# ShinYwings/SingleHDR-tf2

Hardware: AMD Instinct MI355X
Metric: HDR images/sec (512x512) end-to-end inference, deq+lin+hal (higher is better)
Workload: dtype f32

## Files before the change

### include/shdr.h

```cpp
#ifndef SHDR_H_
#define SHDR_H_

#include <stdint.h>

#ifdef __cplusplus
extern "C" {
#endif

void shdr_config_reload(void);

#define SHDR_OK          0
#define SHDR_E_SHAPE    (-1)
#define SHDR_E_ALIGN    (-2)
#define SHDR_E_ARCH     (-3)
#define SHDR_E_LAUNCH   (-4)
#define SHDR_E_NULL     (-5)

#define SHDR_ACT_NONE   0
#define SHDR_ACT_RELU   1
#define SHDR_ACT_LRELU  2
#define SHDR_ACT_TANH   3

#define SHDR_ALGO_AUTO    0
#define SHDR_ALGO_MFMA    1
// ... 55 lines not shown
int shdr_conv2d_plan_f32(const shdr_conv2d_desc* d, int has_residual);
int64_t shdr_conv2d_prepared_filter_elems_f32(const shdr_conv2d_desc* d, int has_residual);
int shdr_conv2d_filter_is_plain_f32(const shdr_conv2d_desc* d, int has_residual);
int shdr_conv2d_prepare_filter_f32(const shdr_conv2d_desc* d, int has_residual, const float* w, float* prepared, void* stream);
int64_t shdr_conv2d_workspace_bytes_f32(const shdr_conv2d_desc* d, int has_residual);
int shdr_conv2d_fwd_prepared_f32(const shdr_conv2d_desc* d, const float* x1, const float* x2, const float* prepared,
                                 const float* bias, const float* scale, const float* shift, const float* residual, float* y,
                                 float* y_pool, void* workspace, void* stream);
int shdr_conv2d_fwd_prepared_ranged_f32(const shdr_conv2d_desc* d, const float* x1, const float* x2, const float* prepared,
                                        const float* bias, const float* scale, const float* shift, const float* residual, float* y,
                                        float* y_pool, void* workspace, const float* x1_range, const float* x2_range, float* y_range,
                                        void* stream);
int shdr_conv2d_projected_ok_f32(const shdr_conv2d_desc* d);
int shdr_conv2d_fwd_prepared_projected_f32(const shdr_conv2d_desc* d, const float* x1, const float* x2, const float* prepared,
                                           const float* bias, const float* scale, const float* shift, const float* proj, float* y_proj,
                                           float* y, float* y_pool, void* workspace, const float* x1_range, const float* x2_range,
                                           float* y_range, void* stream);

int shdr_conv2d_up2_lowres_ok_f32(const shdr_conv2d_desc* d);
int64_t shdr_conv2d_up2_lowres_filter_elems_f32(const shdr_conv2d_desc* d);
int shdr_conv2d_up2_lowres_prepare_filter_f32(const shdr_conv2d_desc* d, const float* w, float* prepared, void* stream);
int64_t shdr_conv2d_up2_lowres_workspace_bytes_f32(const shdr_conv2d_desc* d);
int shdr_conv2d_fwd_up2_lowres_f32(const shdr_conv2d_desc* d, const float* x, const float* prepared, const float* bias,
                                   const float* scale, const float* shift, float* y, void* workspace, const float* x_range,
                                   float* y_range, void* stream);

int shdr_conv2d_up2_fused_ok_f32(const shdr_conv2d_desc* d);
int shdr_conv2d_up2_narrow_enabled(void);
int64_t shdr_conv2d_up2_fused_filter_elems_f32(const shdr_conv2d_desc* d);
int shdr_conv2d_up2_fused_prepare_filter_f32(const shdr_conv2d_desc* d, const float* w, float* prepared, void* stream);
int shdr_conv2d_fwd_up2_fused_f32(const shdr_conv2d_desc* d, const float* x, const float* prepared, const float* bias,
                                  const float* scale, const float* shift, const float* proj, float* y_proj, float* y,
                                  const float* x_range, float* y_range, void* stream);

int shdr_conv2d_wgrad_f32(const shdr_conv2d_desc* d, const float* x, int which, const float* dz,
                          float* dw, void* stream);
int shdr_filter_transform_f32(const float* w, float* wt, int KH, int KW, int Cin, int Cout,
                              int c_begin, int c_count, float scale, void* stream);
int64_t shdr_conv2d_dgrad_workspace_bytes_f32(const shdr_conv2d_desc* d, int which);
int shdr_conv2d_dgrad_f32(const shdr_conv2d_desc* d, int which, const float* dz, const float* w, float* dx, void* workspace,
                          void* stream);
int shdr_conv2d_dgrad_tracks_range_f32(const shdr_conv2d_desc* d, int which);
int shdr_conv2d_dgrad_ranged_f32(const shdr_conv2d_desc* d, int which, const float* dz, const float* w, float* dx, void* workspace,
                                 const float* dz_range, float* dx_range, void* stream);
enum { SHDR_OP_CONV2D_FWD = 0, SHDR_OP_CONV2D_DGRAD = 1, SHDR_OP_CONV2D_WGRAD_WINOGRAD = 2, SHDR_OP_BATCHNORM = 3,
       SHDR_OP_ACT_BWD_BIAS = 4  };
#define SHDR_BN_MAX_BLOCKS 1024
int64_t shdr_workspace_bytes(int op, const shdr_conv2d_desc* d, int arg);
int shdr_bias_grad_f32(const float* dz, float* db, int64_t npix, int C, void* stream);

int shdr_soft_hist_fwd_f32(const float* x, float* y, int64_t npix, int C, int B, void* stream);
int shdr_soft_hist_bwd_f32(const float* x, const float* dy, float* dx, int64_t npix, int C, int B, void* stream);

int shdr_lin_frontend_fwd_f32(const float* img, float* y, int N, int H, int W,
                              int y_channels, void* stream);

int shdr_avgpool2_fwd_f32(const float* x, float* y, int N, int H, int W, int C, void* stream);
int shdr_maxpool2_fwd_f32(const float* x, float* y, int N, int H, int W, int C, void* stream);
int shdr_maxpool3s2_fwd_f32(const float* x, float* y, int N, int H, int W, int C, void* stream);
int shdr_resize2x_fwd_f32(const float* x, float* y, int N, int H, int W, int C, void* stream);
int shdr_gap_fwd_f32(const float* x, float* y, int N, int HW, int C, void* stream);

int shdr_invcrf_decode_fwd_f32(const float* feat, const float* wfc, const float* bfc,
                               const float* table, float* out, int B, int F, int K,
                               void* stream);
int shdr_increase_fwd_f32(const float* rf, float* out, int B, int K, void* stream);
// ... 457 lines not shown
```

### singlehdr-tf2_amd/_lib.py

```python
import ctypes
import os

_HERE = os.path.dirname(os.path.abspath(__file__))
LIB_PATH = os.environ.get("SHDR_LIB") or os.path.join(_HERE, "libshdr.so")

c_int = ctypes.c_int
c_i64 = ctypes.c_int64
c_f32 = ctypes.c_float
c_ptr = ctypes.c_void_p


class ConvDesc(ctypes.Structure):
    _fields_ = [("N", ctypes.c_int32), ("H", ctypes.c_int32), ("W", ctypes.c_int32),
                ("C1", ctypes.c_int32), ("C2", ctypes.c_int32),
                ("Cout", ctypes.c_int32), ("KH", ctypes.c_int32), ("KW", ctypes.c_int32),
                ("stride", ctypes.c_int32), ("pad_t", ctypes.c_int32), ("pad_l", ctypes.c_int32),
                ("Ho", ctypes.c_int32), ("Wo", ctypes.c_int32),
                ("x2_scale", ctypes.c_float),
                ("act1", ctypes.c_int32), ("act2", ctypes.c_int32),
                ("res_cstride", ctypes.c_int32), ("y_cstride", ctypes.c_int32),
                ("algo", ctypes.c_int32), ("cout_valid", ctypes.c_int32),
                ("w_batch_stride", ctypes.c_int64),
                ("y_pix_stride", ctypes.c_int32), ("y_off_h", ctypes.c_int32), ("y_off_w", ctypes.c_int32),
                ("y_H", ctypes.c_int32), ("y_W", ctypes.c_int32),
# ... 72 lines not shown
    "shdr_config_reload": (None, []),
    "shdr_conv2d_x3_input_absmax_f32": (c_int, [c_ptr, c_i64, c_ptr, c_ptr]),
    "shdr_conv2d_x3n_ok_f32": (c_int, [ctypes.POINTER(ConvDesc)]),
    "shdr_conv2d_x3n_filter_elems_f32": (c_i64, [ctypes.POINTER(ConvDesc)]),
    "shdr_conv2d_x3n_prepare_filter_f32": (c_int, [ctypes.POINTER(ConvDesc), c_ptr, c_ptr, c_ptr]),
    "shdr_conv2d_fwd_x3n_f32": (c_int, [ctypes.POINTER(ConvDesc)] + [c_ptr] * 10),
    "shdr_conv2d_fwd_x3n_ranged_f32": (c_int, [ctypes.POINTER(ConvDesc)] + [c_ptr] * 13),
    "shdr_act_bwd_bias_f32": (c_int, [c_ptr, c_ptr, c_ptr, c_ptr, c_ptr, c_i64, c_int, c_int, c_ptr]),
    "shdr_winograd_filter_packed_f32": (c_int, [c_ptr, c_ptr, c_int, c_int, c_ptr]),
    "shdr_conv2d_wgrad_winograd_f32": (c_int, [c_ptr] * 4 + [c_int] * 7 + [c_f32, c_ptr]),
    "shdr_crc32c": (ctypes.c_uint32, [c_ptr, ctypes.c_uint64, ctypes.c_uint32]),
    "shdr_same_pad": (c_int, [c_int, c_int, c_int, ctypes.POINTER(c_int), ctypes.POINTER(c_int)]),
    "shdr_conv2d_fwd_f32": (c_int, [ctypes.POINTER(ConvDesc)] + [c_ptr] * 9),
    "shdr_conv2d_fwd_yrange_f32": (c_int, [ctypes.POINTER(ConvDesc)] + [c_ptr] * 10),
    "shdr_conv2d_plan_f32": (c_int, [ctypes.POINTER(ConvDesc), c_int]),
    "shdr_conv2d_prepared_filter_elems_f32": (c_i64, [ctypes.POINTER(ConvDesc), c_int]),
    "shdr_conv2d_filter_is_plain_f32": (c_int, [ctypes.POINTER(ConvDesc), c_int]),
    "shdr_conv2d_prepare_filter_f32": (c_int, [ctypes.POINTER(ConvDesc), c_int, c_ptr, c_ptr, c_ptr]),
    "shdr_conv2d_workspace_bytes_f32": (c_i64, [ctypes.POINTER(ConvDesc), c_int]),
    "shdr_conv2d_fwd_prepared_f32": (c_int, [ctypes.POINTER(ConvDesc)] + [c_ptr] * 11),
    "shdr_conv2d_fwd_prepared_ranged_f32": (c_int, [ctypes.POINTER(ConvDesc)] + [c_ptr] * 14),
    "shdr_conv2d_projected_ok_f32": (c_int, [ctypes.POINTER(ConvDesc)]),
    "shdr_conv2d_fwd_prepared_projected_f32": (c_int, [ctypes.POINTER(ConvDesc)] + [c_ptr] * 15),
    "shdr_conv2d_up2_lowres_ok_f32": (c_int, [ctypes.POINTER(ConvDesc)]),
    "shdr_conv2d_up2_lowres_filter_elems_f32": (c_i64, [ctypes.POINTER(ConvDesc)]),
    "shdr_conv2d_up2_lowres_prepare_filter_f32": (c_int, [ctypes.POINTER(ConvDesc), c_ptr, c_ptr, c_ptr]),
    "shdr_conv2d_up2_lowres_workspace_bytes_f32": (c_i64, [ctypes.POINTER(ConvDesc)]),
    "shdr_conv2d_fwd_up2_lowres_f32": (c_int, [ctypes.POINTER(ConvDesc)] + [c_ptr] * 10),
    "shdr_conv2d_up2_fused_ok_f32": (c_int, [ctypes.POINTER(ConvDesc)]),
    "shdr_conv2d_up2_narrow_enabled": (c_int, []),
    "shdr_conv2d_up2_fused_filter_elems_f32": (c_i64, [ctypes.POINTER(ConvDesc)]),
    "shdr_conv2d_up2_fused_prepare_filter_f32": (c_int, [ctypes.POINTER(ConvDesc), c_ptr, c_ptr, c_ptr]),
    "shdr_conv2d_fwd_up2_fused_f32": (c_int, [ctypes.POINTER(ConvDesc)] + [c_ptr] * 11),
    "shdr_conv2d_fwd_x3_projected_f32": (c_int, [ctypes.POINTER(ConvDesc)] + [c_ptr] * 14),
    "shdr_conv2d_fwd_x3_residual_f32": (c_int, [ctypes.POINTER(ConvDesc)] + [c_ptr] * 12),
    "shdr_conv2d_dgrad_workspace_bytes_f32": (c_i64, [ctypes.POINTER(ConvDesc), c_int]),
    "shdr_conv2d_dgrad_f32": (c_int, [ctypes.POINTER(ConvDesc), c_int, c_ptr, c_ptr, c_ptr, c_ptr, c_ptr]),
    "shdr_conv2d_dgrad_tracks_range_f32": (c_int, [ctypes.POINTER(ConvDesc), c_int]),
    "shdr_conv2d_dgrad_ranged_f32": (c_int, [ctypes.POINTER(ConvDesc), c_int, c_ptr, c_ptr, c_ptr, c_ptr, c_ptr, c_ptr, c_ptr]),
    "shdr_workspace_bytes": (c_i64, [c_int, ctypes.POINTER(ConvDesc), c_int]),
    "shdr_soft_hist_bwd_f32": (c_int, [c_ptr, c_ptr, c_ptr, c_i64, c_int, c_int, c_ptr]),
    "shdr_conv2d_wgrad_f32": (c_int, [ctypes.POINTER(ConvDesc), c_ptr, c_int, c_ptr, c_ptr, c_ptr]),
    "shdr_filter_transform_f32": (c_int, [c_ptr, c_ptr, c_int, c_int, c_int, c_int, c_int, c_int, c_f32, c_ptr]),
    "shdr_bias_grad_f32": (c_int, [c_ptr, c_ptr, c_i64, c_int, c_ptr]),
    "shdr_soft_hist_fwd_f32": (c_int, [c_ptr, c_ptr, c_i64, c_int, c_int, c_ptr]),
    "shdr_lin_frontend_fwd_f32": (c_int, [c_ptr, c_ptr, c_int, c_int, c_int, c_int, c_ptr]),
    "shdr_avgpool2_fwd_f32": (c_int, [c_ptr, c_ptr, c_int, c_int, c_int, c_int, c_ptr]),
    "shdr_maxpool2_fwd_f32": (c_int, [c_ptr, c_ptr, c_int, c_int, c_int, c_int, c_ptr]),
    "shdr_maxpool3s2_fwd_f32": (c_int, [c_ptr, c_ptr, c_int, c_int, c_int, c_int, c_ptr]),
    "shdr_resize2x_fwd_f32": (c_int, [c_ptr, c_ptr, c_int, c_int, c_int, c_int, c_ptr]),
    "shdr_gap_fwd_f32": (c_int, [c_ptr, c_ptr, c_int, c_int, c_int, c_ptr]),
    "shdr_invcrf_decode_fwd_f32": (c_int, [c_ptr] * 5 + [c_int, c_int, c_int, c_ptr]),
    "shdr_increase_fwd_f32": (c_int, [c_ptr, c_ptr, c_int, c_int, c_ptr]),
    "shdr_apply_rf_fwd_f32": (c_int, [c_ptr, c_ptr, c_ptr, c_int, c_i64, c_int, c_ptr]),
    "shdr_clip_fwd_f32": (c_int, [c_ptr, c_ptr, c_i64, c_f32, c_f32, c_ptr]),
    "shdr_vgg_preprocess_fwd_f32": (c_int, [c_ptr, c_ptr, c_i64, c_int, c_ptr]),
    "shdr_reverse3_fwd_f32": (c_int, [c_ptr, c_ptr, c_i64, c_ptr]),
    "shdr_alpha_blend_fwd_f32": (c_int, [c_ptr, c_ptr, c_ptr, c_ptr, c_i64, c_f32, c_ptr]),
    "shdr_pack3_fwd_f32": (c_int, [c_ptr] * 4 + [c_int, c_ptr, c_int, c_i64, c_ptr]),
    "shdr_logc_fwd_f32": (c_int, [c_ptr, c_ptr, c_i64, c_ptr]),
    "shdr_affine_act_f32": (c_int, [c_ptr] * 5 + [c_i64, c_int, c_int, c_ptr]),
    "shdr_pad_channels_f32": (c_int, [c_ptr, c_ptr, c_i64, c_int, c_int, c_ptr]),
    "shdr_act_bwd_f32": (c_int, [c_ptr, c_ptr, c_ptr, c_i64, c_int, c_ptr]),
    "shdr_clip_bwd_f32": (c_int, [c_ptr, c_ptr, c_ptr, c_i64, c_f32, c_f32, c_ptr]),
    "shdr_add_f32": (c_int, [c_ptr, c_ptr, c_ptr, c_i64, c_ptr]),
    "shdr_add_ranged_f32": (c_int, [c_ptr, c_ptr, c_ptr, c_i64, c_ptr, c_ptr]),
# ... 115 lines not shown
```

### singlehdr-tf2_amd/_ops.py

```python
import collections
import ctypes
import math

import numpy as np
import torch

try:
    from . import _lib
except ImportError:
    import _lib

AUTOGRAD = None


def _needs_grad(*tensors):
    return AUTOGRAD is not None and torch.is_grad_enabled() and any(
        isinstance(t, torch.Tensor) and t.requires_grad for t in tensors)


WINOGRAD = True


ACT_NONE, ACT_RELU, ACT_LRELU, ACT_TANH = 0, 1, 2, 3
ALGO_AUTO, ALGO_MFMA, ALGO_DIRECT, ALGO_MFMA_REG = 0, 1, 2, 3
# ... 270 lines not shown


def _conv2d_up2_fused(x, w, bias, act1, scale, shift, act2, proj=None, want_y=None):
    if proj is not None and _d(w).shape[-1] != 64:
        return None
    layer = _up2_layer("fused", x, w, bias, act1, scale, shift, act2)
    if layer is None:
        return None
    lib = _lib.load()
    x_in = x
    d, x, prepared = layer
    if proj is not None:
        proj = _chk(_d(proj), "proj")
        if tuple(proj.shape) != (3, d.Cout):
            raise ValueError("conv2d_up2: proj must be [3, %d]" % d.Cout)
    if want_y is None:
        want_y = proj is None
    xr = _range_of(x_in)
    if xr is None:
        RANGE_MISSES[(tuple(x.shape), None, tuple(_d(w).shape))] += 1
        xr = _new_slot(x.device)
        _lib.check(lib.shdr_absmax_f32(_ptr(x), x.numel(), _ptr(xr), _stream()), "shdr_absmax_f32")
    out = torch.empty((d.N, d.H, d.W, d.Cout), device=x.device, dtype=torch.float32) if want_y else None
    yj = torch.empty((d.N, d.H, d.W, 3), device=x.device, dtype=torch.float32) if proj is not None else None
    yr = _new_slot(x.device) if want_y else None
    rc = lib.shdr_conv2d_fwd_up2_fused_f32(ctypes.byref(d), _ptr(x), _ptr(prepared), _ptr(_d(bias)), _ptr(_d(scale)), _ptr(_d(shift)),
                                           _ptr(proj), _ptr(yj), _ptr(out), _ptr(xr), _ptr(yr), _stream())
    _lib.check(rc, "shdr_conv2d_fwd_up2_fused_f32")
    if proj is not None:
        PROJECTED_LAUNCHES[0] += 1
    if want_y:
        _set_range(out, yr)
    return out if proj is None else ((yj, out) if want_y else yj)


def _conv2d_raw(x, w, bias, stride, x2, x2_scale, act1, scale, shift, residual, act2, algo, out, cout_valid, pad, out_hw,
                w_batch_stride, pool, prologue=0, proj=None):
    lib = _lib.load()
    x_in, x2_in = x, x2
    x = _chk(_d(x), "x")
    w_var = w
    w = _chk(_d(w), "w")
    n, h, wd, c1 = x.shape
    if prologue == PROLOGUE_BILINEAR2X:
        h, wd = 2 * h, 2 * wd
    kh, kw, cin, cout_gemm = w.shape
    cout = cout_gemm if cout_valid is None else int(cout_valid)
    c2 = 0
    if x2 is not None:
        x2 = _chk(_d(x2), "x2")
        if x2.shape[:3] != x.shape[:3]:
            raise ValueError("conv2d: x2 spatial shape %s != x %s" % (tuple(x2.shape), tuple(x.shape)))
        c2 = x2.shape[3]
    if cin != c1 + c2:
        raise ValueError("conv2d: filter expects %d input channels, got %d+%d" % (cin, c1, c2))
    ho, pt = same_pad(h, kh, stride)
    wo, pl = same_pad(wd, kw, stride)
    if pad is not None:
        pt, pl = pad
    if out_hw is not None:
        ho, wo = out_hw
    d = _lib.ConvDesc()
    d.N, d.H, d.W, d.C1, d.C2 = n, h, wd, c1, c2
    d.Cout, d.KH, d.KW, d.stride = cout_gemm, kh, kw, stride
    d.cout_valid = cout
    d.pad_t, d.pad_l, d.Ho, d.Wo = pt, pl, ho, wo
# ... 2234 lines not shown
```

### singlehdr-tf2_amd/build.py

```python
import glob
import os
import shutil
import subprocess
import sys

HERE = os.path.dirname(os.path.abspath(__file__))
CSRC = os.path.join(HERE, "csrc")
INCLUDE = os.path.normpath(os.path.join(HERE, "..", "include"))
OBJ_DIR = os.path.join(HERE, "build")
LIB = os.path.join(HERE, "libshdr.so")

SOURCES = {
    "api.cpp": [],
    "conv.hip": [],
    "conv_plan.hip": [],
    "conv_x3.hip": [],
    "conv_x3n.hip": [],
    "conv_f16.hip": [],
    "conv_f16_patch.hip": [],
    "conv_f16_w3.hip": [],
    "wgrad_x3.hip": [],
    "wgrad_f16.hip": [],
    "wgrad_f16_alltaps.hip": [],
    "elem_f16.hip": ["-ffp-contract=off"],
    "wgrad.hip": [],
    "wgrad_winograd.hip": [],
    "bwd.hip": [],
    "finetune.hip": [],
    "winograd.hip": [],
    "winograd_fused.hip": [],
    "frontend.hip": ["-ffp-contract=off"],
    "pool.hip": [],
    "up2_lowres.hip": [],
    "up2_fused.hip": [],
    "crf.hip": [],
    "glue.hip": [],
    "imageio.hip": [],
    "hdr_rle.hip": [],
    "hdr_rle_dec.hip": [],
    "metrics.hip": [],
    "camera.hip": ["-ffp-contract=off"],
    "dataset.hip": ["-ffp-contract=off"],
    "exr.hip": ["-ffp-contract=off"],
    "exr_write.hip": ["-ffp-contract=off"],
    "deflate.hip": [],
    "deflate_lz.hip": [],
    "inflate.hip": [],
    "piz.hip": [],
    "piz_enc.hip": [],
    "hdr_real.hip": ["-ffp-contract=off"],
    "jpeg.hip": ["-ffp-contract=off"],
    "jpeg_scan.hip": [],
    "jpeg_enc.hip": ["-ffp-contract=off"],
}
COMMON = ["-O3", "-std=c++17", "-fPIC", "--offload-arch=gfx950", "-I" + INCLUDE, "-I" + CSRC,
          "-Wall", "-Wno-unused-function"]


def _hipcc():
    for cand in (os.environ.get("HIPCC"), shutil.which("hipcc"), "/opt/rocm/bin/hipcc"):
        if cand and os.path.exists(cand):
            return cand
    raise RuntimeError("hipcc not found (set HIPCC)")


def _stale(target, deps):
    if not os.path.exists(target):
# ... 34 lines not shown
```

### singlehdr-tf2_amd/linearization_net.py

```python
import os

import numpy as np
import torch

try:
    from . import _ops as K
    from ._layers import Layer, Conv2D, BatchNormalization, Dense, is_training, taping
except ImportError:
    import _ops as K
    from _layers import Layer, Conv2D, BatchNormalization, Dense, is_training, taping

_HERE = os.path.dirname(os.path.abspath(__file__))
FRONTEND_CHANNELS = 93
FRONTEND_CHANNELS_PADDED = 96


def _conv_bn(conv, norm, x, relu, residual=None, cin_pad=None, training=False):
    if is_training(training):
        z = conv(x) if cin_pad is None else conv.call_padded(x, cin_pad=cin_pad)
        if residual is None:
            return norm.train_apply(z, relu=relu)
        y = norm.train_apply(z, relu=False)
        return K.AUTOGRAD.add_relu(residual, y) if relu else K.add(residual, y)
    if taping(x, residual, conv.kernel, conv.bias, norm.gamma, norm.beta):
# ... 12 lines not shown
        super().__init__()
        s = strides if isinstance(strides, int) else strides[0]
        self.conv1 = Conv2D(in_channels, branch1_filter, 1, s, use_bias=False, device=device)
        self.norm1 = BatchNormalization(branch1_filter, device=device)
        self.conv2 = Conv2D(in_channels, branch2_filters[0], 1, s, use_bias=False, device=device)
        self.norm2 = BatchNormalization(branch2_filters[0], device=device)
        self.conv3 = Conv2D(branch2_filters[0], branch2_filters[1], 3, 1, use_bias=False, device=device)
        self.norm3 = BatchNormalization(branch2_filters[1], device=device)
        self.conv4 = Conv2D(branch2_filters[1], branch2_filters[2], 1, 1, use_bias=False, device=device)
        self.norm4 = BatchNormalization(branch2_filters[2], device=device)

    def call(self, x, training="training"):
        t = training
        x, xb = K.fork(x)
        norm1 = _conv_bn(self.conv1, self.norm1, x, relu=False, training=t)
        act2 = _conv_bn(self.conv2, self.norm2, xb, relu=True, training=t)
        act3 = _conv_bn(self.conv3, self.norm3, act2, relu=True, training=t)
        return _conv_bn(self.conv4, self.norm4, act3, relu=True, residual=norm1, training=t)


class resBlock_type2(Layer):

    def __init__(self, in_channels, filters, device=None):
        super().__init__()
        self.conv1 = Conv2D(in_channels, filters[0], 1, 1, use_bias=False, device=device)
        self.norm1 = BatchNormalization(filters[0], device=device)
        self.conv2 = Conv2D(filters[0], filters[1], 3, 1, use_bias=False, device=device)
        self.norm2 = BatchNormalization(filters[1], device=device)
        self.conv3 = Conv2D(filters[1], filters[2], 1, 1, use_bias=False, device=device)
        self.norm3 = BatchNormalization(filters[2], device=device)

    def call(self, x, training="training"):
        t = training
        x, xb = K.fork(x)
        act1 = _conv_bn(self.conv1, self.norm1, xb, relu=True, training=t)
        act2 = _conv_bn(self.conv2, self.norm2, act1, relu=True, training=t)
        return _conv_bn(self.conv3, self.norm3, act2, relu=True, residual=x, training=t)


class crfFeatureNet(Layer):

    def __init__(self, padding="SAME", device=None):
        super().__init__()
        self.conv1 = Conv2D(FRONTEND_CHANNELS, 64, (7, 7), (2, 2), device=device)
        self.norm1 = BatchNormalization(64, device=device)
        self.res1 = resBlock_type1(64, 256, [64, 64, 256], (1, 1), device=device)
        self.res2 = resBlock_type2(256, [64, 64, 256], device=device)
        self.res3 = resBlock_type2(256, [64, 64, 256], device=device)
        self.res4 = resBlock_type1(256, 512, [128, 128, 512], (2, 2), device=device)
        self.res5 = resBlock_type2(512, [128, 128, 512], device=device)

    def call(self, ldr, training="training"):
        cin = ldr.shape[-1]
        x = _conv_bn(self.conv1, self.norm1, ldr, relu=True,
                     cin_pad=None if cin == FRONTEND_CHANNELS else cin, training=training)
        x = K.maxpool3s2(x)
        x = self.res1(x, training)
        x = self.res2(x, training)
        x = self.res3(x, training)
        x = self.res4(x, training)
        x = self.res5(x, training)
        return K.global_avg_pool(x)


def load_invemor_table(device):
    if os.path.exists("invemor.txt"):
# ... 53 lines not shown
```

Before: 951.0.

## Fuse ResNet bottleneck (1x1-3x3-1x1 + BN + residual) into one kernel

```diff
diff --git a/include/shdr.h b/include/shdr.h
--- a/include/shdr.h
+++ b/include/shdr.h
@@ -111,6 +111,14 @@
 int shdr_conv2d_fwd_up2_fused_f32(const shdr_conv2d_desc* d, const float* x, const float* prepared, const float* bias,
                                   const float* scale, const float* shift, const float* proj, float* y_proj, float* y,
                                   const float* x_range, float* y_range, void* stream);
+
+int shdr_resnet_bottleneck_ok_f32(int N, int H, int W, int C, int Cm);
+int64_t shdr_resnet_bottleneck_filter_elems_f32(int C, int Cm);
+int shdr_resnet_bottleneck_prepare_filter_f32(int C, int Cm, const float* w1, const float* w2, const float* w3, float* prepared,
+                                              void* stream);
+int shdr_resnet_bottleneck_fwd_f32(int N, int H, int W, int C, int Cm, const float* x, const float* prepared, const float* scale1,
+                                   const float* shift1, const float* scale2, const float* shift2, const float* scale3,
+                                   const float* shift3, float* y, const float* x_range, float* y_range, void* stream);
 
 int shdr_conv2d_wgrad_f32(const shdr_conv2d_desc* d, const float* x, int which, const float* dz,
                           float* dw, void* stream);
diff --git a/singlehdr-tf2_amd/_lib.py b/singlehdr-tf2_amd/_lib.py
--- a/singlehdr-tf2_amd/_lib.py
+++ b/singlehdr-tf2_amd/_lib.py
@@ -128,6 +128,10 @@
     "shdr_conv2d_up2_fused_filter_elems_f32": (c_i64, [ctypes.POINTER(ConvDesc)]),
     "shdr_conv2d_up2_fused_prepare_filter_f32": (c_int, [ctypes.POINTER(ConvDesc), c_ptr, c_ptr, c_ptr]),
     "shdr_conv2d_fwd_up2_fused_f32": (c_int, [ctypes.POINTER(ConvDesc)] + [c_ptr] * 11),
+    "shdr_resnet_bottleneck_ok_f32": (c_int, [c_int] * 5),
+    "shdr_resnet_bottleneck_filter_elems_f32": (c_i64, [c_int] * 2),
+    "shdr_resnet_bottleneck_prepare_filter_f32": (c_int, [c_int] * 2 + [c_ptr] * 5),
+    "shdr_resnet_bottleneck_fwd_f32": (c_int, [c_int] * 5 + [c_ptr] * 12),
     "shdr_conv2d_fwd_x3_projected_f32": (c_int, [ctypes.POINTER(ConvDesc)] + [c_ptr] * 14),
     "shdr_conv2d_fwd_x3_residual_f32": (c_int, [ctypes.POINTER(ConvDesc)] + [c_ptr] * 12),
     "shdr_conv2d_dgrad_workspace_bytes_f32": (c_i64, [ctypes.POINTER(ConvDesc), c_int]),
diff --git a/singlehdr-tf2_amd/_ops.py b/singlehdr-tf2_amd/_ops.py
--- a/singlehdr-tf2_amd/_ops.py
+++ b/singlehdr-tf2_amd/_ops.py
@@ -326,6 +326,63 @@
     if want_y:
         _set_range(out, yr)
     return out if proj is None else ((yj, out) if want_y else yj)
+
+
+def bottleneck(x, w1, scale1, shift1, w2, scale2, shift2, w3, scale3, shift3, fallback=True):
+    y = None
+    if not _is_h(x) and _AUTO_ALGO[PRECISION] == ALGO_AUTO and WINOGRAD and not EXACT_FP32 \
+            and not _needs_grad(x, w1, scale1, shift1, w2, scale2, shift2, w3, scale3, shift3):
+        y = _bottleneck_fused(x, w1, scale1, shift1, w2, scale2, shift2, w3, scale3, shift3)
+    if y is not None or not fallback:
+        return y
+    t = conv2d(x, w1, scale=scale1, shift=shift1, act2=ACT_RELU)
+    t = conv2d(t, w2, scale=scale2, shift=shift2, act2=ACT_RELU)
+    return conv2d(t, w3, scale=scale3, shift=shift3, residual=x, act2=ACT_RELU)
+
+
+def _bottleneck_fused(x, w1, scale1, shift1, w2, scale2, shift2, w3, scale3, shift3):
+    lib = _lib.load()
+    x_in = x
+    x = _d(x)
+    ws = [_d(w) for w in (w1, w2, w3)]
+    if x.dim() != 4 or any(w.dim() != 4 for w in ws):
+        return None
+    n, h, wd, c = x.shape
+    cm = ws[0].shape[3]
+    if [tuple(w.shape) for w in ws] != [(1, 1, c, cm), (3, 3, cm, cm), (1, 1, cm, c)]:
+        return None
+    if not int(lib.shdr_resnet_bottleneck_ok_f32(n, h, wd, c, cm)):
+        return None
+    _chk(x, "x")
+    for w in ws:
+        _chk(w, "w")
+    consts = []
+    for t, nm, ln in ((scale1, "scale1", cm), (shift1, "shift1", cm), (scale2, "scale2", cm), (shift2, "shift2", cm),
+                      (scale3, "scale3", c), (shift3, "shift3", c)):
+        if t is None or _chk(_d(t), nm).numel() != ln:
+            raise ValueError("bottleneck: %s must have %d elements" % (nm, ln))
+        consts.append(_d(t))
+    persistent = all(_is_persistent(w) for w in (w1, w2, w3))
+    nprep = int(lib.shdr_resnet_bottleneck_filter_elems_f32(c, cm))
+    key = ("bottleneck", c, cm, nprep, w2.data_ptr(), w2._version, w3.data_ptr(), w3._version)
+    prepared = _filter_cache_get(w1, "_shdr_packed", key) if persistent else None
+    if prepared is None:
+        prepared = torch.empty(nprep, device=x.device, dtype=torch.float32)
+        _lib.check(lib.shdr_resnet_bottleneck_prepare_filter_f32(c, cm, _ptr(ws[0]), _ptr(ws[1]), _ptr(ws[2]), _ptr(prepared), _stream()),
+                   "shdr_resnet_bottleneck_prepare_filter_f32")
+        if persistent:
+            _filter_cache_put(w1, "_shdr_packed", key, prepared)
+    xr = _range_of(x_in)
+    if xr is None:
+        RANGE_MISSES[(tuple(x.shape), None, tuple(ws[0].shape))] += 1
+        xr = _new_slot(x.device)
+        _lib.check(lib.shdr_absmax_f32(_ptr(x), x.numel(), _ptr(xr), _stream()), "shdr_absmax_f32")
+    out = torch.empty((n, h, wd, c), device=x.device, dtype=torch.float32)
+    yr = _new_slot(x.device)
+    rc = lib.shdr_resnet_bottleneck_fwd_f32(n, h, wd, c, cm, _ptr(x), _ptr(prepared), *[_ptr(t) for t in consts], _ptr(out), _ptr(xr),
+                                            _ptr(yr), _stream())
+    _lib.check(rc, "shdr_resnet_bottleneck_fwd_f32")
+    return _set_range(out, yr)
 
 
 def _conv2d_raw(x, w, bias, stride, x2, x2_scale, act1, scale, shift, residual, act2, algo, out, cout_valid, pad, out_hw,
diff --git a/singlehdr-tf2_amd/build.py b/singlehdr-tf2_amd/build.py
--- a/singlehdr-tf2_amd/build.py
+++ b/singlehdr-tf2_amd/build.py
@@ -33,6 +33,7 @@
     "pool.hip": [],
     "up2_lowres.hip": [],
     "up2_fused.hip": [],
+    "bottleneck_x3.hip": [],
     "crf.hip": [],
     "glue.hip": [],
     "imageio.hip": [],
diff --git a/singlehdr-tf2_amd/csrc/bottleneck_x3.hip b/singlehdr-tf2_amd/csrc/bottleneck_x3.hip
--- /dev/null
+++ b/singlehdr-tf2_amd/csrc/bottleneck_x3.hip
@@ -0,0 +1,481 @@
+#include <hip/hip_fp16.h>
+#include <stdlib.h>
+
+#include <type_traits>
+
+#include "shdr_internal.h"
+
+namespace {
+
+using f32x4 = __attribute__((ext_vector_type(4))) float;
+using f16x8 = __attribute__((ext_vector_type(8))) _Float16;
+
+constexpr int BK_HEADER_FLOATS = 16;
+constexpr int BK_IMG_HALVES = 64 * 32, BK_UNIT_HALVES = 2 * BK_IMG_HALVES;
+constexpr int BK_ROWS = 8;
+constexpr int BK_XSTRIDE = 40;
+
+template <int CM, int TH_>
+struct BKG {
+  static constexpr int C = 4 * CM;
+  static constexpr int TH = TH_;
+  static constexpr int PH = TH + 2, PW = 18, PPIX = PH * PW;
+  static constexpr int NG = (PPIX + 15) / 16;
+  static constexpr int WC = CM / 32;
+  static constexpr int WR = TH / 4;
+  static constexpr int NW = WC * WR, THREADS = 64 * NW;
+  static constexpr int GPW = (NG + WR - 1) / WR;
+  static constexpr int TSTRIDE = CM + 8;
+  static constexpr int XIMG = NG * 16 * BK_XSTRIDE;
+  static constexpr int T1IMG = PPIX * TSTRIDE, T2IMG = TH * 16 * TSTRIDE;
+  static constexpr int PJ = (PPIX * 8 + THREADS - 1) / THREADS;
+  static constexpr int LDS_HALVES = 4 * XIMG > 2 * T1IMG ? 4 * XIMG : 2 * T1IMG;
+  static constexpr int LDS_BYTES = LDS_HALVES * 2;
+  static_assert(WR * 4 == TH && NW <= 8 && T2IMG <= T1IMG, "tile geometry");
+};
+
+struct BKArgs {
+  const float* x;
+  float* y;
+  const _Float16* wp1;
+  const _Float16* wp2;
+  const _Float16* wp3;
+  const float* hdr1;
+  const float* hdr2;
+  const float* hdr3;
+  const float* scale1;
+  const float* shift1;
+  const float* scale2;
+  const float* shift2;
+  const float* scale3;
+  const float* shift3;
+  const unsigned* xr;
+  unsigned* yr;
+  int N, H, W, tiles_x, tiles_y;
+};
+
+__device__ __forceinline__ void bk_range_scale(unsigned b, float& xs, float& ixs) {
+  xs = 1.0f;
+  ixs = 1.0f;
+  if (b != 0u && b < 0x7f800000u) {
+    int ex;
+    frexpf(__uint_as_float(b), &ex);
+    int T = 11 - ex;
+    T = T < -126 ? -126 : (T > 126 ? 126 : T);
+    xs = ldexpf(1.0f, T);
+    ixs = ldexpf(1.0f, -T);
+  }
+}
+__device__ __forceinline__ void bk_split4(const f32x4 v, float xs, unsigned (&h)[2], unsigned (&l)[2]) {
+  const float k2048 = 2048.0f;
+#pragma unroll
+  for (int p = 0; p < 2; ++p) {
+    float t0, t1;
+    asm("v_fma_mixlo_f16 %0, %1, %2, 0" : "=v"(h[p]) : "v"(v[2 * p]), "s"(xs));
+    asm("v_fma_mixhi_f16 %0, %1, %2, 0" : "+v"(h[p]) : "v"(v[2 * p + 1]), "s"(xs));
+    asm("v_fma_mix_f32 %0, %1, %2, -%3 op_sel_hi:[0,0,1]" : "=v"(t0) : "v"(v[2 * p]), "s"(xs), "v"(h[p]));
+    asm("v_fma_mix_f32 %0, %1, %2, -%3 op_sel:[0,0,1] op_sel_hi:[0,0,1]" : "=v"(t1) : "v"(v[2 * p + 1]), "s"(xs), "v"(h[p]));
+    asm("v_fma_mixlo_f16 %0, %1, %2, 0" : "=v"(l[p]) : "v"(t0), "s"(k2048));
+    asm("v_fma_mixhi_f16 %0, %1, %2, 0" : "+v"(l[p]) : "v"(t1), "s"(k2048));
+  }
+}
+__device__ __forceinline__ int bk_xcd_remap(int bid, int nwg) {
+  const int q = nwg >> 3, r = nwg & 7, xcd = bid & 7, idx = bid >> 3;
+  return (xcd < r ? xcd * (q + 1) : r * (q + 1) + (xcd - r) * q) + idx;
+}
+template <int NW>
+__device__ __forceinline__ unsigned bk_block_max(float m, unsigned* words, int lane, int wave) {
+#pragma unroll
+  for (int off = 32; off > 0; off >>= 1) m = fmaxf(m, __shfl_xor(m, off, 64));
+  if (lane == 0) words[wave] = __float_as_uint(m);
+  __syncthreads();
+  unsigned b = words[0];
+#pragma unroll
+  for (int k = 1; k < NW; ++k) b = words[k] > b ? words[k] : b;
+  return __builtin_amdgcn_readfirstlane(b);
+}
+
+struct BKFrag {
+  f16x8 h[2], l[2];
+};
+__device__ __forceinline__ void bk_load_frag(BKFrag& f, const _Float16* g) {
+#pragma unroll
+  for (int k = 0; k < 2; ++k) {
+    f.h[k] = *reinterpret_cast<const f16x8*>(g + k * 16 * 32);
+    f.l[k] = *reinterpret_cast<const f16x8*>(g + BK_IMG_HALVES + k * 16 * 32);
+  }
+}
+template <int NR>
+__device__ __forceinline__ void bk_unit(f32x4 (&acc)[NR][2], const BKFrag& f, const _Float16* ph, const _Float16* pl, int pitch, int ntiles) {
+  f16x8 ws[2];
+#pragma unroll
+  for (int k = 0; k < 2; ++k) ws[k] = f.h[k] * (_Float16)(1.0f / 2048.0f);
+#pragma unroll
+  for (int i = 0; i < NR; ++i) {
+    if (i >= ntiles) break;
+    const f16x8 bh = *reinterpret_cast<const f16x8*>(ph + i * pitch);
+    const f16x8 bl = *reinterpret_cast<const f16x8*>(pl + i * pitch);
+#pragma unroll
+    for (int k = 0; k < 2; ++k) acc[i][k] = __builtin_amdgcn_mfma_f32_16x16x32_f16(f.h[k], bh, acc[i][k], 0, 0, 0);
+#pragma unroll
+    for (int k = 0; k < 2; ++k) acc[i][k] = __builtin_amdgcn_mfma_f32_16x16x32_f16(ws[k], bl, acc[i][k], 0, 0, 0);
+#pragma unroll
+    for (int k = 0; k < 2; ++k) acc[i][k] = __builtin_amdgcn_mfma_f32_16x16x32_f16(f.l[k], bh, acc[i][k], 0, 0, 0);
+  }
+}
+
+template <int CM, int TH>
+__global__ __launch_bounds__((BKG<CM, TH>::THREADS), (BKG<CM, TH>::NW == 8 ? 1 : 2)) void bottleneck_x3_kernel(const BKArgs a) {
+  using G = BKG<CM, TH>;
+  constexpr int C = G::C, PW = G::PW, PPIX = G::PPIX, NG = G::NG, WC = G::WC, TS = G::TSTRIDE, PJ = G::PJ, NW = G::NW, GPW = G::GPW;
+  constexpr int BK_THREADS = G::THREADS;
+  constexpr int XIMG = G::XIMG, T1IMG = G::T1IMG, T2IMG = G::T2IMG;
+  constexpr int NCH_A = C / 32, NCH_B = CM / 32;
+  extern __shared__ __attribute__((aligned(16))) _Float16 bsm[];
+  __shared__ unsigned bk_words[3][8];
+
+  const int tid = threadIdx.x, lane = tid & 63;
+  const int wave = __builtin_amdgcn_readfirstlane(tid >> 6);
+  const int fi = lane & 15, fg = lane >> 4;
+  const int wc = wave % WC, wr = wave / WC;
+  int L = bk_xcd_remap(blockIdx.x, gridDim.x);
+  const int tx = L % a.tiles_x; L /= a.tiles_x;
+  const int ty = L % a.tiles_y;
+  const int img = L / a.tiles_y;
+  const int oh0 = ty * TH, ow0 = tx * 16;
+  const int frag_lane = fi * 32 + 8 * fg;
+
+  f32x4 t1v[GPW][2];
+  float xs1, ixs1;
+  {
+    int ppix[PJ], pdst[PJ];
+#pragma unroll
+    for (int j = 0; j < PJ; ++j) {
+      const int id = tid + BK_THREADS * j;
+      const int pp = id >> 3, q = id & 7;
+      const int py = pp / PW, px = pp - py * PW;
+      const int ih = oh0 - 1 + py, iw = ow0 - 1 + px;
+      const bool in = pp < PPIX && (unsigned)ih < (unsigned)a.H && (unsigned)iw < (unsigned)a.W;
+      ppix[j] = in ? (img * a.H + ih) * a.W + iw : -1;
+      pdst[j] = pp < PPIX ? pp * BK_XSTRIDE + 4 * q : -1;
+    }
+    using Set0 = std::integral_constant<int, 0>;
+    using Set1 = std::integral_constant<int, 1>;
+    f32x4 pr_sets[2][PJ];
+    auto load_patch = [&](int c, auto setc) __attribute__((always_inline)) {
+      constexpr int S = decltype(setc)::value;
+#pragma unroll
+      for (int j = 0; j < PJ; ++j) {
+        pr_sets[S][j] = (f32x4){0.f, 0.f, 0.f, 0.f};
+        if (ppix[j] >= 0) pr_sets[S][j] = *reinterpret_cast<const f32x4*>(a.x + (size_t)(unsigned)ppix[j] * C + (c << 5) + 4 * (tid & 7));
+      }
+    };
+    float xs = 1.0f, ixs = 1.0f;
+    auto store_patch = [&](int buf, auto setc) __attribute__((always_inline)) {
+      constexpr int S = decltype(setc)::value;
+#pragma unroll
+      for (int j = 0; j < PJ; ++j) {
+        if (pdst[j] < 0) continue;
+        unsigned h[2], l[2];
+        bk_split4(pr_sets[S][j], xs, h, l);
+        *reinterpret_cast<uint2*>(bsm + buf * 2 * XIMG + pdst[j]) = make_uint2(h[0], h[1]);
+        *reinterpret_cast<uint2*>(bsm + buf * 2 * XIMG + XIMG + pdst[j]) = make_uint2(l[0], l[1]);
+      }
+    };
+    const _Float16* w1 = a.wp1 + (size_t)(wc >> 1) * NCH_A * BK_UNIT_HALVES + (wc & 1) * 32 * 32 + frag_lane;
+    const int g0 = GPW * wr;
+    const int ngrp = NG - g0 < GPW ? NG - g0 : GPW;
+    const int rd = (g0 * 16 + fi) * BK_XSTRIDE + 8 * fg;
+#pragma unroll
+    for (int i = 0; i < GPW; ++i)
+#pragma unroll
+      for (int k = 0; k < 2; ++k) t1v[i][k] = (f32x4){0.f, 0.f, 0.f, 0.f};
+    BKFrag fa, fb;
+    load_patch(0, Set0{});
+    load_patch(1, Set1{});
+    bk_load_frag(fa, w1);
+    bk_range_scale(*a.xr, xs, ixs);
+    xs = __uint_as_float(__builtin_amdgcn_readfirstlane(__float_as_uint(xs)));
+    store_patch(0, Set0{});
+    load_patch(2, Set0{});
+    auto chunk = [&](int c, auto nxt, const BKFrag& cur, BKFrag& other) __attribute__((always_inline)) {
+      __syncthreads();
+      if (c + 1 < NCH_A) {
+        bk_load_frag(other, w1 + (size_t)(c + 1) * BK_UNIT_HALVES);
+        store_patch((c + 1) & 1, nxt);
+        if (c + 3 < NCH_A) load_patch(c + 3, nxt);
+      }
+      const _Float16* ph = bsm + (c & 1) * 2 * XIMG + rd;
+      bk_unit<GPW>(t1v, cur, ph, ph + XIMG, 16 * BK_XSTRIDE, ngrp);
+    };
+#pragma unroll 1
+    for (int c = 0; c < NCH_A; c += 2) {
+      chunk(c, Set1{}, fa, fb);
+      chunk(c + 1, Set0{}, fb, fa);
+    }
+    const float inv = a.hdr1[1] * ixs;
+    float m = 0.0f;
+#pragma unroll
+    for (int k = 0; k < 2; ++k) {
+      const int co = 16 * (2 * wc + k) + 4 * fg;
+      const f32x4 sc = *reinterpret_cast<const f32x4*>(a.scale1 + co), sh = *reinterpret_cast<const f32x4*>(a.shift1 + co);
+#pragma unroll
+      for (int i = 0; i < GPW; ++i) {
+        const int pp = (g0 + i) * 16 + fi;
+        const int py = pp / PW, px = pp - py * PW;
+        const bool in = pp < PPIX && (unsigned)(oh0 - 1 + py) < (unsigned)a.H && (unsigned)(ow0 - 1 + px) < (unsigned)a.W;
+        f32x4 v = t1v[i][k] * inv;
+        asm("" : "+v"(v));
+        v = v * sc + sh;
+#pragma unroll
+        for (int e = 0; e < 4; ++e) {
+          v[e] = in ? fmaxf(v[e], 0.0f) : 0.0f;
+          m = fmaxf(m, v[e]);
+        }
+        t1v[i][k] = v;
+      }
+    }
+    const unsigned b1 = bk_block_max<NW>(m, bk_words[0], lane, wave);
+    bk_range_scale(b1, xs1, ixs1);
+    xs1 = __uint_as_float(__builtin_amdgcn_readfirstlane(__float_as_uint(xs1)));
+#pragma unroll
+    for (int i = 0; i < GPW; ++i) {
+      const int pp = (g0 + i) * 16 + fi;
+      if (pp >= PPIX) continue;
+#pragma unroll
+      for (int k = 0; k < 2; ++k) {
+        unsigned h[2], l[2];
+        bk_split4(t1v[i][k], xs1, h, l);
+        const int dst = pp * TS + 16 * (2 * wc + k) + 4 * fg;
+        *reinterpret_cast<uint2*>(bsm + dst) = make_uint2(h[0], h[1]);
+        *reinterpret_cast<uint2*>(bsm + T1IMG + dst) = make_uint2(l[0], l[1]);
+      }
+    }
+  }
+  __syncthreads();
+
+  const int row0 = 4 * wr;
+  const int ow = ow0 + fi;
+  f32x4 acc[4][2];
+  float xs2, ixs2;
+  {
+#pragma unroll
+    for (int i = 0; i < 4; ++i)
+#pragma unroll
+      for (int k = 0; k < 2; ++k) acc[i][k] = (f32x4){0.f, 0.f, 0.f, 0.f};
+    constexpr int NU = NCH_B * 9;
+    const _Float16* w2 = a.wp2 + (size_t)(wc >> 1) * NU * BK_UNIT_HALVES + (wc & 1) * 32 * 32 + frag_lane;
+    const int rd = (row0 * PW + fi) * TS + 8 * fg;
+    BKFrag fr[2];
+    bk_load_frag(fr[0], w2);
+#pragma unroll 1
+    for (int c = 0; c < NCH_B; c += 2) {
+#pragma unroll
+      for (int u = 0; u < 18; ++u) {
+        const int cc = c + u / 9, tap = u % 9;
+        const int un = cc * 9 + tap;
+        if (un + 1 < NU) bk_load_frag(fr[(u + 1) & 1], w2 + (size_t)(un + 1) * BK_UNIT_HALVES);
+        const _Float16* ph = bsm + rd + ((tap / 3) * PW + tap % 3) * TS + 32 * cc;
+        bk_unit<4>(acc, fr[u & 1], ph, ph + T1IMG, PW * TS, 4);
+      }
+    }
+    const float inv = a.hdr2[1] * ixs1;
+    float m = 0.0f;
+#pragma unroll
+    for (int k = 0; k < 2; ++k) {
+      const int co = 16 * (2 * wc + k) + 4 * fg;
+      const f32x4 sc = *reinterpret_cast<const f32x4*>(a.scale2 + co), sh = *reinterpret_cast<const f32x4*>(a.shift2 + co);
+#pragma unroll
+      for (int i = 0; i < 4; ++i) {
+        const bool in = oh0 + row0 + i < a.H && ow < a.W;
+        f32x4 v = acc[i][k] * inv;
+        asm("" : "+v"(v));
+        v = v * sc + sh;
+#pragma unroll
+        for (int e = 0; e < 4; ++e) {
+          v[e] = in ? fmaxf(v[e], 0.0f) : 0.0f;
+          m = fmaxf(m, v[e]);
+        }
+        acc[i][k] = v;
+      }
+    }
+    const unsigned b2 = bk_block_max<NW>(m, bk_words[1], lane, wave);
+    bk_range_scale(b2, xs2, ixs2);
+    xs2 = __uint_as_float(__builtin_amdgcn_readfirstlane(__float_as_uint(xs2)));
+#pragma unroll
+    for (int i = 0; i < 4; ++i)
+#pragma unroll
+      for (int k = 0; k < 2; ++k) {
+        unsigned h[2], l[2];
+        bk_split4(acc[i][k], xs2, h, l);
+        const int dst = ((row0 + i) * 16 + fi) * TS + 16 * (2 * wc + k) + 4 * fg;
+        *reinterpret_cast<uint2*>(bsm + dst) = make_uint2(h[0], h[1]);
+        *reinterpret_cast<uint2*>(bsm + T2IMG + dst) = make_uint2(l[0], l[1]);
+      }
+  }
+  __syncthreads();
+
+  {
+    const float inv = a.hdr3[1] * ixs2;
+    const unsigned yr_seen = a.yr ? __hip_atomic_load(a.yr, __ATOMIC_RELAXED, __HIP_MEMORY_SCOPE_AGENT) : 0u;
+    const int rd = (row0 * 16 + fi) * TS + 8 * fg;
+    const bool col_ok = ow < a.W;
+    float ym = 0.0f;
+    constexpr int NPASS = C / (32 * WC);
+    auto w3_of = [&](int g) __attribute__((always_inline)) {
+      return a.wp3 + (size_t)(g >> 2) * NCH_B * BK_UNIT_HALVES + (g & 3) * 16 * 32 + frag_lane;
+    };
+    BKFrag fr[2];
+    bk_load_frag(fr[0], w3_of(2 * wc));
+#pragma unroll 1
+    for (int s = 0; s < NPASS; ++s) {
+      const int g = s * 2 * WC + 2 * wc;
+      const _Float16* w3 = w3_of(g);
+      int rds = rd;
+      if constexpr (CM == 128) asm volatile("" : "+v"(rds));
+      f32x4 res[4][2], sc[2], sh[2];
+#pragma unroll
+      for (int k = 0; k < 2; ++k) {
+        const int co = 16 * (g + k) + 4 * fg;
+        sc[k] = *reinterpret_cast<const f32x4*>(a.scale3 + co);
+        sh[k] = *reinterpret_cast<const f32x4*>(a.shift3 + co);
+#pragma unroll
+        for (int i = 0; i < 4; ++i) {
+          const int oh = oh0 + row0 + i;
+          res[i][k] = (oh < a.H && col_ok) ? *reinterpret_cast<const f32x4*>(a.x + ((size_t)(img * a.H + oh) * a.W + ow) * C + co) : (f32x4){0.f, 0.f, 0.f, 0.f};
+        }
+      }
+#pragma unroll
+      for (int i = 0; i < 4; ++i)
+#pragma unroll
+        for (int k = 0; k < 2; ++k) acc[i][k] = (f32x4){0.f, 0.f, 0.f, 0.f};
+#pragma unroll
+      for (int c = 0; c < NCH_B; ++c) {
+        if (c + 1 < NCH_B) bk_load_frag(fr[(c + 1) & 1], w3 + (size_t)(c + 1) * BK_UNIT_HALVES);
+        else if (s + 1 < NPASS) bk_load_frag(fr[0], w3_of(g + 2 * WC));
+        const _Float16* ph = bsm + rds + 32 * c;
+        bk_unit<4>(acc, fr[c & 1], ph, ph + T2IMG, 16 * TS, 4);
+      }
+#pragma unroll
+      for (int i = 0; i < 4; ++i) {
+        const int oh = oh0 + row0 + i;
+        if (oh >= a.H) continue;
+#pragma unroll
+        for (int k = 0; k < 2; ++k) {
+          f32x4 v = acc[i][k] * inv;
+          asm("" : "+v"(v));
+          v = v * sc[k] + sh[k];
+          v += res[i][k];
+#pragma unroll
+          for (int e = 0; e < 4; ++e) v[e] = fmaxf(v[e], 0.0f);
+          if (col_ok) {
+            *reinterpret_cast<f32x4*>(a.y + ((size_t)(img * a.H + oh) * a.W + ow) * C + 16 * (g + k) + 4 * fg) = v;
+            ym = fmaxf(fmaxf(fmaxf(fmaxf(ym, fabsf(v[0])), fabsf(v[1])), fabsf(v[2])), fabsf(v[3]));
+          }
+        }
+      }
+    }
+    if (a.yr) {
+      const unsigned b = bk_block_max<NW>(ym, bk_words[2], lane, wave);
+      if (tid == 0 && b > yr_seen) atomicMax(a.yr, b);
+    }
+  }
+}
+
+bool bk_shape_ok(int N, int H, int W, int C, int Cm) {
+  return N > 0 && H > 0 && W > 0 && (Cm == 64 || Cm == 128) && C == 4 * Cm && (long)N * H * W < (1L << 31);
+}
+long bk_blocks(int N, int H, int W) { return (long)N * ((H + BK_ROWS - 1) / BK_ROWS) * ((W + 15) / 16); }
+void bk_descs(int C, int Cm, shdr_conv2d_desc (&d)[3]) {
+  for (int i = 0; i < 3; ++i) {
+    d[i] = shdr_conv2d_desc{};
+    d[i].N = 1; d[i].H = 16; d[i].W = 16; d[i].Ho = 16; d[i].Wo = 16; d[i].stride = 1; d[i].x2_scale = 1.0f;
+    d[i].KH = d[i].KW = i == 1 ? 3 : 1;
+    d[i].pad_t = d[i].pad_l = i == 1 ? 1 : 0;
+    d[i].C1 = i == 0 ? C : Cm;
+    d[i].Cout = i == 2 ? C : Cm;
+    d[i].cout_valid = d[i].Cout; d[i].y_cstride = d[i].Cout;
+  }
+}
+
+template <int CM, int TH>
+int bk_launch(const BKArgs& a, hipStream_t st) {
+  constexpr int lds = BKG<CM, TH>::LDS_BYTES;
+  static_assert(lds <= 160 * 1024 - 256, "the images of a block must fit the CU's LDS");
+  static bool attr_done[shdr::kMaxDevices] = {};
+  const int dev_slot = shdr::device_slot();
+  if (!attr_done[dev_slot]) {
+    hipError_t e = hipFuncSetAttribute(reinterpret_cast<const void*>(&bottleneck_x3_kernel<CM, TH>), hipFuncAttributeMaxDynamicSharedMemorySize, lds);
+    if (e != hipSuccess) return shdr::fail(SHDR_E_ARCH, "hipFuncSetAttribute: %s", hipGetErrorString(e));
+    attr_done[dev_slot] = true;
+  }
+  const long nblk = (long)a.N * a.tiles_y * a.tiles_x;
+  hipLaunchKernelGGL((bottleneck_x3_kernel<CM, TH>), dim3((unsigned)nblk), dim3(BKG<CM, TH>::THREADS), lds, st, a);
+  return shdr::check_launch("bottleneck_x3_kernel");
+}
+
+}
+
+extern "C" int shdr_resnet_bottleneck_ok_f32(int N, int H, int W, int C, int Cm) {
+  if (!bk_shape_ok(N, H, W, C, Cm) || SHDR_ENV("SHDR_NO_BOTTLENECK_FUSED") != nullptr || SHDR_ENV("SHDR_NO_WINOGRAD") != nullptr ||
+      SHDR_ENV("SHDR_NO_X3") != nullptr || SHDR_ENV("SHDR_NO_X3_1X1") != nullptr)
+    return 0;
+  long min_blocks = 128;
+  if (const char* e = SHDR_ENV("SHDR_BOTTLENECK_MIN_BLOCKS")) min_blocks = atol(e);
+  const long nblk = bk_blocks(N, H, W);
+  return nblk >= min_blocks && nblk <= 0x7fffffffL ? 1 : 0;
+}
+
+extern "C" int64_t shdr_resnet_bottleneck_filter_elems_f32(int C, int Cm) {
+  if (!bk_shape_ok(1, 1, 1, C, Cm)) return -1;
+  shdr_conv2d_desc d[3];
+  bk_descs(C, Cm, d);
+  int64_t total = 0;
+  for (int i = 0; i < 3; ++i) {
+    const int64_t n = shdr_conv2d_x3_filter_elems_f32(&d[i]);
+    if (n < 0) return -1;
+    total += n;
+  }
+  return total;
+}
+extern "C" int shdr_resnet_bottleneck_prepare_filter_f32(int C, int Cm, const float* w1, const float* w2, const float* w3, float* prepared,
+                                                         void* stream) {
+  SHDR_REQUIRE(w1 && w2 && w3 && prepared, SHDR_E_NULL, "resnet_bottleneck_prepare_filter: null pointer");
+  SHDR_REQUIRE(bk_shape_ok(1, 1, 1, C, Cm), SHDR_E_SHAPE, "resnet_bottleneck_prepare_filter: need Cm 64 or 128 and C = 4 Cm");
+  shdr_conv2d_desc d[3];
+  bk_descs(C, Cm, d);
+  const float* w[3] = {w1, w2, w3};
+  float* out = prepared;
+  for (int i = 0; i < 3; ++i) {
+    if (int rc = shdr_conv2d_x3_prepare_filter_f32(&d[i], w[i], out, stream)) return rc;
+    out += shdr_conv2d_x3_filter_elems_f32(&d[i]);
+  }
+  return SHDR_OK;
+}
+
+extern "C" int shdr_resnet_bottleneck_fwd_f32(int N, int H, int W, int C, int Cm, const float* x, const float* prepared, const float* scale1,
+                                              const float* shift1, const float* scale2, const float* shift2, const float* scale3,
+                                              const float* shift3, float* y, const float* x_range, float* y_range, void* stream) {
+  SHDR_REQUIRE(x && prepared && y && x_range && scale1 && shift1 && scale2 && shift2 && scale3 && shift3, SHDR_E_NULL,
+               "resnet_bottleneck: null x / prepared filter / y / x_range / BatchNorm constants");
+  SHDR_REQUIRE(shdr_resnet_bottleneck_ok_f32(N, H, W, C, Cm), SHDR_E_SHAPE, "resnet_bottleneck: block not taken (shdr_resnet_bottleneck_ok_f32)");
+  SHDR_REQUIRE(x != y, SHDR_E_SHAPE, "resnet_bottleneck: y must not alias x");
+  SHDR_REQUIRE(shdr::aligned16(x) && shdr::aligned16(prepared) && shdr::aligned16(y) && shdr::aligned16(scale1) && shdr::aligned16(shift1) &&
+                   shdr::aligned16(scale2) && shdr::aligned16(shift2) && shdr::aligned16(scale3) && shdr::aligned16(shift3),
+               SHDR_E_ALIGN, "resnet_bottleneck: tensors must be 16-byte aligned");
+  shdr_conv2d_desc d[3];
+  bk_descs(C, Cm, d);
+  BKArgs a{};
+  a.x = x; a.y = y;
+  const float* p = prepared;
+  a.hdr1 = p; a.wp1 = reinterpret_cast<const _Float16*>(p + BK_HEADER_FLOATS); p += shdr_conv2d_x3_filter_elems_f32(&d[0]);
+  a.hdr2 = p; a.wp2 = reinterpret_cast<const _Float16*>(p + BK_HEADER_FLOATS); p += shdr_conv2d_x3_filter_elems_f32(&d[1]);
+  a.hdr3 = p; a.wp3 = reinterpret_cast<const _Float16*>(p + BK_HEADER_FLOATS);
+  a.scale1 = scale1; a.shift1 = shift1; a.scale2 = scale2; a.shift2 = shift2; a.scale3 = scale3; a.shift3 = shift3;
+  a.xr = reinterpret_cast<const unsigned*>(x_range); a.yr = reinterpret_cast<unsigned*>(y_range);
+  a.N = N; a.H = H; a.W = W;
+  a.tiles_x = (W + 15) / 16;
+  a.tiles_y = (H + BK_ROWS - 1) / BK_ROWS;
+  hipStream_t st = shdr::stream_of(stream);
+  return Cm == 64 ? bk_launch<64, BK_ROWS>(a, st) : bk_launch<128, BK_ROWS>(a, st);
+}
diff --git a/singlehdr-tf2_amd/linearization_net.py b/singlehdr-tf2_amd/linearization_net.py
--- a/singlehdr-tf2_amd/linearization_net.py
+++ b/singlehdr-tf2_amd/linearization_net.py
@@ -68,6 +68,11 @@
 
     def call(self, x, training="training"):
         t = training
+        layers = ((self.conv1, self.norm1), (self.conv2, self.norm2), (self.conv3, self.norm3))
+        if not is_training(t) and not taping(x, *(v for c, n in layers for v in (c.kernel, n.gamma, n.beta))):
+            y = K.bottleneck(x, *(v for c, n in layers for v in (c.kernel,) + n.folded()), fallback=False)
+            if y is not None:
+                return y
         x, xb = K.fork(x)
         act1 = _conv_bn(self.conv1, self.norm1, xb, relu=True, training=t)
         act2 = _conv_bn(self.conv2, self.norm2, act1, relu=True, training=t)
```

After: 952.5, median of 4. No clear change (+0.2%).
